# KMS-TEAM/vi_slam

Measured on AMD Instinct MI355X. Metric: frames/sec ORB extract+match, higher is better.
Workload: dtype u8; 1 GPU; kitti00_mono_1241x376_n1000; nfeatures=1000, nlevels=8, contexts_in_flight=4, distinct_frames=32, match=SearchForInitialization(prev frame) window 100

## Files before the change

vi_slam_amd/csrc/vslam_ctx.h:

```cpp
#ifndef VSLAM_CTX_H
#define VSLAM_CTX_H
#include <hip/hip_runtime.h>

#include <algorithm>
#include <atomic>
#include <cmath>
#include <condition_variable>
#include <cstdio>
#include <cstring>
#include <functional>
#include <mutex>
#include <string>
#include <thread>
#include <vector>

#include "../../include/vslam_orb_pattern.h"
#include "vslam_host.h"
#include "vslam_pool.h"
#include "vslam_kernels.h"
#include "vslam_tuning.h"

std::string& vslam_err();
#define g_err (vslam_err())

// ... 159 lines not shown
    double rgbd_ms = 0;
    long rgbd_passes = 0;
    hipEvent_t ev_lp[3] = {};
    bool lp_timed = false;
    double lp_ms[2] = {0, 0};
    long lp_passes = 0;

    bool dev_octree = false;
    OctParams oct;
    uint32_t* d_pts = nullptr;
    uint8_t* d_oct_sorted = nullptr;
    uint32_t* d_oct_lut = nullptr;
    int32_t* d_oct_redo = nullptr;
    uint32_t* d_sel_xyr = nullptr;
    int32_t* d_sel_cnt = nullptr;
    int32_t* d_counts = nullptr;
    int32_t* h_counts = nullptr;
    bool cand_on_host = false;
    int last_nimg = 0;

    bool profiling = false;
    hipEvent_t ev_prof[10] = {};
    double prof_ms[5] = {0, 0, 0, 0, 0};
    long prof_batches = 0, prof_images = 0;

    WorkerPool* pool = nullptr;
};


static inline int vslam_pix_bpp(int fmt) { return fmt == VSLAM_PIX_GRAY8 ? 1 : fmt <= VSLAM_PIX_BGR8 ? 3 : 4; }
// ... 44 lines not shown
```

vi_slam_amd/csrc/vslam_device.h:

```cpp
#ifndef VSLAM_DEVICE_H
#define VSLAM_DEVICE_H

#include <hip/hip_runtime.h>
#include <stdint.h>

#include "../../include/vslam_fe.h"

#define VSLAM_EDGE 19
#define VSLAM_BORDER 16
#define VSLAM_HALF_PATCH 15

struct LevelGeom {
    int32_t w, h;
    int32_t pitch;
    uint32_t off;
    float scale;
    int32_t pad[3];
};

struct PyramidGeom {
    int32_t nlevels;
    int32_t pad[3];
    LevelGeom lv[VSLAM_MAX_LEVELS];
};
// ... 33 lines not shown
    int32_t nIni[VSLAM_MAX_LEVELS];
    float hX[VSLAM_MAX_LEVELS];
    int32_t cellFirst[VSLAM_MAX_LEVELS + 1];
    int32_t selOff[VSLAM_MAX_LEVELS];
    int32_t selStride;
    int32_t maxNodes;
    int32_t ptsCap;
    int32_t maxIter;
    void* dbg;
    int32_t fineD[VSLAM_MAX_LEVELS];
    int32_t lutOff[VSLAM_MAX_LEVELS];
    int32_t lutW[VSLAM_MAX_LEVELS];
    int32_t fineLdsOff;
    int32_t fineLdsBytes;
    const uint32_t* lut;
};

struct StereoJob {
    const vslam_kp* kpsL;
    const uint8_t* descL;
    const vslam_kp* kpsR;
    const uint8_t* descR;
    const int32_t* cntL;
    const int32_t* cntR;
    int32_t slotL, slotR;
};
#define VSLAM_MAX_STEREO_JOBS 32
struct StereoJobs {
    StereoJob job[VSLAM_MAX_STEREO_JOBS];
};
// ... 169 lines not shown
```

vi_slam_amd/csrc/vslam_fe.hip:

```cpp
#if defined(__SSE2__)
#include <emmintrin.h>
#endif
#include "vslam_ctx.h"

#include <algorithm>
#include <chrono>
#include <mutex>
#include <cstdio>
#include <cstdlib>

void vslam_host_prof_report();

std::string& vslam_err() {
    static thread_local std::string e;
    return e;
}
extern "C" const char* vslam_last_error(void) { return vslam_err().c_str(); }

static std::mutex g_gate_mu;

static void gate_unlink(vslam_fe* fe) {
    if (fe->fast_gate) {
        auto& w = fe->fast_gate->gate_waiters;
        w.erase(std::remove(w.begin(), w.end(), fe), w.end());
// ... 29 lines not shown
    hipFree(fe->d_pattern);
    if (fe->h_top2) hipHostFree(fe->h_top2);
    hipFree(fe->d_part);
    hipFree(fe->d_idx2);
    hipFree(fe->d_dist2);
    hipFree(fe->d_dmat);
    hipFree(fe->d_tmp_desc[0]);
    hipFree(fe->d_tmp_desc[1]);
    hipFree(fe->d_stereo);
    hipFree(fe->d_pts);
    hipFree(fe->d_oct_sorted);
    hipFree(fe->d_oct_lut);
    hipFree(fe->d_sel_xyr);
    hipFree(fe->d_oct_redo);
    hipFree(fe->d_sel_cnt);
    if (fe->h_stereo) hipHostFree(fe->h_stereo);
    if (!fe->init_in_block) hipFree(fe->d_init);
    hipFree(fe->d_init_scratch);
    hipFree(fe->d_ukps);
    hipFree(fe->d_proj);
    hipFree(fe->d_sbp);
    if (fe->h_sbp) hipHostFree(fe->h_sbp);
    hipFree(fe->d_x3dw);
    hipFree(fe->d_mpflags);
    if (fe->h_proj) hipHostFree(fe->h_proj);
    if (fe->h_img) hipHostFree(fe->h_img);
    if (fe->h_depth) hipHostFree(fe->h_depth);
    hipFree(fe->d_stage);
    if (fe->graph_exec) hipGraphExecDestroy(fe->graph_exec);
    hipFree(fe->d_bow);
// ... 274 lines not shown
    fe->oct_threads = fe->tune.oct_threads == 256 || fe->tune.oct_threads == 512 || fe->tune.oct_threads == 1024
                          ? fe->tune.oct_threads
                          : fe->B <= 2 ? 1024 : 256;
    if (!on_device) return VSLAM_OK;
    if (vk_octree_set_max_lds((size_t)O.fineLdsOff + (size_t)O.fineLdsBytes + 16) != 0) {
        g_err = "hipFuncSetAttribute(k_octree, max dynamic LDS) failed";
        return VSLAM_ERR_HIP;
    }
    const size_t np = (size_t)fe->B * fe->cand_cap;
    HIPCHK(hipMalloc((void**)&fe->d_pts, np * 4));
    HIPCHK(hipMalloc((void**)&fe->d_sel_xyr, (size_t)fe->B * O.selStride * 4));
    HIPCHK(hipMalloc((void**)&fe->d_sel_cnt, (size_t)fe->B * VSLAM_MAX_LEVELS * 4));
    HIPCHK(hipMalloc((void**)&fe->d_oct_sorted, np * 8));
    HIPCHK(hipMalloc((void**)&fe->d_oct_redo, (size_t)fe->B * VSLAM_MAX_LEVELS * 4));
    HIPCHK(hipMemset(fe->d_oct_redo, 0, (size_t)fe->B * VSLAM_MAX_LEVELS * 4));
    UPLOAD(fe->d_oct_lut, plan.lut.data(), plan.lut.size() * 4);
    O.lut = fe->d_oct_lut;
    return VSLAM_OK;
}

static int create_stream_and_pool(vslam_fe* fe) {
    const int pr = tune_or(fe->tune.stream_priority, 0);
    int lo = 0, hi = 0;
    if (pr != 0 && hipDeviceGetStreamPriorityRange(&lo, &hi) == hipSuccess && lo != hi)
        HIPCHK(hipStreamCreateWithPriority(&fe->stream, hipStreamNonBlocking, pr == 1 ? lo : hi));
    else
        HIPCHK(hipStreamCreateWithFlags(&fe->stream, hipStreamNonBlocking));
    HIPCHK(hipEventCreateWithFlags(&fe->ev_cand, hipEventDisableTiming));
    fe->use_graph = fe->tune.graphs != 0;
    fe->sel_level.resize((size_t)fe->B * fe->p.nlevels);
// ... 397 lines not shown
        if (fe->pix_fmt != VSLAM_PIX_GRAY8) {
            vk_gray_images(st, ds, fe->d_pyr, fe->slot_stride, fe->geom.lv[0].off, fe->geom.lv[0].pitch, p.width, p.height, nimg,
                           0, fe->pix_fmt, fe->gray_shift, fe->tune);
            src_at_slots(fe, nimg);
        }
    } else {
        if (on_device != VSLAM_IMGS_STAGED) {
            int rc = upload_host_rows(fe, nimg, imgs, pitch, on_device);
            if (rc) return rc;
        }
        src_at_slots(fe, nimg);
    }
    fe->last_nimg = nimg;
    fe->cand_on_host = false;
    int32_t* d_errw = fe->dev_octree ? fe->d_counts + (size_t)fe->B * 4 : nullptr;
    if (fe->pyr_groups.empty()) vk_reset_headers(st, fe->d_cand, fe->cand_stride, nimg, d_errw);
    const bool prof = fe->profiling;
    if (prof) HIPCHK(hipEventRecord(fe->ev_prof[0], st));
    bool first_group = true;
    for (const auto& g : fe->pyr_groups) {
        vk_pyramid_group(st, fe->d_pyr, fe->slot_stride, fe->src, g.dev, g.lds_bytes, nimg,
                         first_group ? fe->d_cand : nullptr, fe->cand_stride, first_group ? d_errw : nullptr);
        first_group = false;
    }
    for (int l = 1; l < L && fe->pyr_groups.empty(); l++) {
        if (fe->d_quads[l])
            vk_resize_level_v2(st, fe->d_pyr, fe->slot_stride, fe->src, fe->geom.lv[l - 1], fe->geom.lv[l], l - 1,
                               fe->d_qbase[l], fe->d_quads[l], fe->d_ytab[l], fe->d_yb[l], nimg);
        else
            vk_resize_level(st, fe->d_pyr, fe->slot_stride, fe->src, fe->geom.lv[l - 1], fe->geom.lv[l], l - 1,
                            fe->d_xtab[l], fe->d_xa[l], fe->d_ytab[l], fe->d_yb[l], nimg);
    }
    if (prof) HIPCHK(hipEventRecord(fe->ev_prof[1], st));
    if (fe->fast_gate && fe->fast_gate->ev_fast) HIPCHK(hipStreamWaitEvent(st, fe->fast_gate->ev_fast, 0));
    if (fe->nbands > 0 && tune_or(fe->tune.fast_kernel, fe->B <= 2 ? 3 : 4) != 3)
        vk_fast_bands(st, fe->d_pyr, fe->slot_stride, fe->src, fe->geom, fe->d_bands, fe->nbands, fe->d_band_classes, fe->d_cells,
                      (int)fe->cells.size(), fe->d_cand, fe->cand_stride, p.ini_th_fast, p.min_th_fast, fe->band_max_wh, fe->band_max_iw, nimg);
// ... 91 lines not shown
    HIPCHK(hipMemcpyAsync(fe->d_counts, fe->h_counts, (size_t)(fe->B * 4 + 4) * 4, hipMemcpyHostToDevice, st));
    HIPCHK(hipMemcpyAsync(fe->d_sel, fe->h_sel, (size_t)nimg * fe->cap * sizeof(SelKp), hipMemcpyHostToDevice, st));
    if (fe->profiling) {
        HIPCHK(hipEventRecord(fe->ev_prof[7], st));
        HIPCHK(hipEventRecord(fe->ev_prof[8], st));
    }
    return VSLAM_OK;
}

static int select_dev(vslam_fe* fe, int nimg, int lap0, int lap1) {
    hipStream_t st = fe->stream;
    int32_t* d_err = fe->d_counts + (size_t)fe->B * 4;
    const int rc = enqueue_blur(fe, nimg);
    if (rc) return rc;
    if (fe->profiling) HIPCHK(hipEventRecord(fe->ev_prof[7], st));
    vk_octree(st, fe->d_cand, fe->cand_stride, (int)fe->cells.size(), fe->oct, fe->d_pts,
              fe->d_oct_sorted, (size_t)fe->cand_cap, fe->d_sel_xyr, fe->d_sel_cnt, d_err, fe->p.nlevels, nimg,
              fe->d_oct_redo, fe->tune.oct_regkeys, fe->oct_threads);
    vk_assign_out(st, fe->oct, fe->geom, fe->d_sel_xyr, fe->d_sel_cnt, lap0, lap1, fe->d_sel, fe->d_counts, fe->cap,
                  d_err, nimg, fe->d_oct_redo);
    if (fe->profiling) HIPCHK(hipEventRecord(fe->ev_prof[8], st));
    return VSLAM_OK;
}

static int enqueue_back(vslam_fe* fe, int nimg, int lap0, int lap1) {
    hipStream_t st = fe->stream;
    const bool prof = fe->profiling;
    int rc = fe->dev_octree ? select_dev(fe, nimg, lap0, lap1) : select_host(fe, nimg, lap0, lap1);
    if (rc) return rc;
    if (prof) HIPCHK(hipEventRecord(fe->ev_prof[5], st));
    vk_orient_describe_dev(st, fe->d_pyr, fe->d_blur, fe->slot_stride, fe->src, fe->geom, fe->d_sel, fe->d_counts,
                           fe->d_pattern, fe->d_kps, fe->d_desc, fe->cap, (fe->p.flags & VSLAM_FLAG_ATAN_FMA) ? 1 : 0,
                           nimg, fe->tune.desc_kpw >= 0 ? fe->tune.desc_kpw : fe->desc_kpw_hint);
    rc = vslam_enqueue_undistort(fe, nimg);
    if (rc) return rc;
// ... 610 lines not shown
```

vi_slam_amd/csrc/vslam_image_kernels.hip:

```cpp
#include "vslam_kernels.h"
#include "vslam_wave.h"

__device__ __forceinline__ const uint8_t* level_base_v2(const uint8_t* pyr, size_t slot_stride,
                                                        const BatchSrc& src, const LevelGeom& lg, int level,
                                                        int slot, int* pitch) {
    if (level == 0) {
        *pitch = (int)src.pitch0[slot];
        return src.l0[slot];
    }
    *pitch = lg.pitch;
    return pyr + (size_t)slot * slot_stride + lg.off;
}

__device__ __forceinline__ int refl101_v2(int p, int len) {
    if (p < 0) p = -p;
    if (p >= len) p = 2 * (len - 1) - p;
    return min(max(p, 0), len - 1);
}

#define BV_OUTW 248

__device__ __forceinline__ uint32_t udot4(uint32_t a, uint32_t b, uint32_t c) {
    return __builtin_amdgcn_udot4(a, b, c, false);
}
// ... 281 lines not shown
};
__device__ __forceinline__ PyrTileU pyr_tile_uniform(const PyrTileDev& t) {
    PyrTileU u;
#define PTU(f) u.f = __builtin_amdgcn_readfirstlane((int)t.f)
    PTU(c0); PTU(nc); PTU(r0); PTU(nr); PTU(sq0); PTU(sq1); PTU(sr0); PTU(sr1);
#undef PTU
    u.lds_off = (uint32_t)__builtin_amdgcn_readfirstlane((int)t.lds_off);
    u.pitch = (uint32_t)__builtin_amdgcn_readfirstlane((int)t.pitch);
    u.rt_off = (uint32_t)__builtin_amdgcn_readfirstlane((int)t.rt_off);
    return u;
}

template <int NT>
__global__ void __launch_bounds__(NT)
k_pyramid_group(uint8_t* pyr, size_t slot_stride, BatchSrc src, PyrGroupDev G, int nslots, uint8_t* reset_cand,
                size_t cand_stride, int32_t* reset_err) {
    extern __shared__ __align__(16) uint8_t psm[];
    constexpr int NW = NT / 64;
    const int lane = threadIdx.x & 63;
    const int wave = __builtin_amdgcn_readfirstlane((int)(threadIdx.x >> 6));
    if (reset_cand && blockIdx.x == 0) {
        if ((int)threadIdx.x < nslots) *(uint2*)(reset_cand + (size_t)threadIdx.x * cand_stride) = make_uint2(0u, 0u);
        if (reset_err && threadIdx.x < 4) reset_err[threadIdx.x] = 0;
    }
    const int nwork = G.ntiles * nslots, per_xcd = (nwork + 7) >> 3;
    const int wk = (int)(blockIdx.x & 7) * per_xcd + (int)(blockIdx.x >> 3);
    if (wk >= nwork) return;
    const int slot = wk / G.ntiles, tile = wk - slot * G.ntiles;
    const PyrTileDev* T = G.tiles + (size_t)tile * (G.nl + 1);
    const PyrTileDev S0 = T[0];
    if (S0.nr <= 0 || S0.nc <= 0) return;

    uint4 qsel[VSLAM_PYR_GROUP_LEVELS], qcf[VSLAM_PYR_GROUP_LEVELS];
    int qloc[VSLAM_PYR_GROUP_LEVELS];
#pragma unroll
    for (int j = 1; j <= VSLAM_PYR_GROUP_LEVELS; j++) {
        qsel[j - 1] = qcf[j - 1] = make_uint4(0, 0, 0, 0);
        qloc[j - 1] = 0;
// ... 89 lines not shown
                const uint32_t v0 = (uint32_t)(((__mul24(b0, g0) >> 16) + (__mul24(b1, hp0) >> 16) + 2) >> 2);
                const uint32_t v1 = (uint32_t)(((__mul24(b0, g1) >> 16) + (__mul24(b1, hp1) >> 16) + 2) >> 2);
                const uint32_t v2 = (uint32_t)(((__mul24(b0, g2) >> 16) + (__mul24(b1, hp2) >> 16) + 2) >> 2);
                const uint32_t v3 = (uint32_t)(((__mul24(b0, g3) >> 16) + (__mul24(b1, hp3) >> 16) + 2) >> 2);
                const uint32_t out = (v0 & 0xFF) | ((v1 & 0xFF) << 8) | ((v2 & 0xFF) << 16) | (v3 << 24);
                *(uint32_t*)(psm + dbase + __mul24(r, dp)) = out;
                if (qstore && r >= D.sr0 && r < D.sr1) *(uint32_t*)(gout + (size_t)r * gpitch) = out;
            }
#undef PYR_HPASS
        }
        __syncthreads();
    }
}

void vk_pyramid_group(hipStream_t st, uint8_t* pyr, size_t slot_stride, const BatchSrc& src, const PyrGroupDev& G,
                      size_t lds_bytes, int nslots, uint8_t* reset_cand, size_t cand_stride, int32_t* reset_err) {
    const int nwork = G.ntiles * nslots;
    hipLaunchKernelGGL(k_pyramid_group<256>, dim3(((nwork + 7) / 8) * 8), dim3(256), lds_bytes, st, pyr, slot_stride, src, G, nslots,
                       reset_cand, cand_stride, reset_err);
}

typedef unsigned short ushort2v __attribute__((ext_vector_type(2)));
__device__ __forceinline__ uint32_t pk_sub_sat(uint32_t a, uint32_t b) {
    uint32_t r;
    asm("v_pk_sub_u16 %0, %1, %2 clamp" : "=v"(r) : "v"(a), "v"(b));
    return r;
}
__device__ __forceinline__ uint32_t pk_add(uint32_t a, uint32_t b) {
    uint32_t r;
    asm("v_pk_add_u16 %0, %1, %2" : "=v"(r) : "v"(a), "v"(b));
    return r;
}
__device__ __forceinline__ uint32_t pk_min(uint32_t a, uint32_t b) {
    uint32_t r;
// ... 783 lines not shown
```

vi_slam_amd/csrc/vslam_kernels.h:

```cpp
#ifndef VSLAM_KERNELS_H
#define VSLAM_KERNELS_H

#include "vslam_tuning.h"
#include "vslam_device.h"

void vk_upload_disc(const int umax[16]);

void vk_resize_level(hipStream_t st, uint8_t* pyr, size_t slot_stride, const BatchSrc& src,
                     const LevelGeom& sg, const LevelGeom& dg, int src_level, const uint16_t* xtab,
                     const int16_t* xa, const uint16_t* ytab, const int16_t* yb, int nslots);

void vk_hamming_matrix(hipStream_t st, const uint8_t* q, int nq, const uint8_t* t, int nt, uint8_t* out);
int vk_hamming_top2_batch_split(int nprob, int max_nq, int max_nt);
void vk_hamming_top2_batch(hipStream_t st, const Top2Jobs& jobs, int nprob, int max_nq, int nrows, int nsplit, uint32_t* part,
                           int32_t* idx2, int32_t* dist2);

void vk_blur7_v2(hipStream_t st, const uint8_t* pyr, size_t slot_stride, const BatchSrc& src, const PyramidGeom& g,
                 uint8_t* blur, const uint32_t* tasks, int ntasks, const int32_t taps[7], int rows_per_task,
                 int nslots);
void vk_pyramid_group(hipStream_t st, uint8_t* pyr, size_t slot_stride, const BatchSrc& src, const PyrGroupDev& G,
                      size_t lds_bytes, int nslots, uint8_t* reset_cand = nullptr, size_t cand_stride = 0,
                      int32_t* reset_err = nullptr);
void vk_fast_cells_v3(hipStream_t st, const uint8_t* pyr, size_t slot_stride, const BatchSrc& src,
                      const PyramidGeom& g, const CellDesc* cells, int ncells, uint8_t* cand_region,
                      size_t cand_stride, int iniTh, int minTh, int tile_rows, int max_window_w, int max_px, int nslots);
int vk_fast_bands_check(int max_wh, int max_iw, int max_cells_per_band);
void vk_fast_bands(hipStream_t st, const uint8_t* pyr, size_t slot_stride, const BatchSrc& src, const PyramidGeom& g,
                   const BandDesc* bands, int nbands, const uint8_t* classes, const CellDesc* cells, int ncells, uint8_t* cand_region,
                   size_t cand_stride, int iniTh, int minTh, int max_wh, int max_iw, int nslots);
void vk_resize_level_v2(hipStream_t st, uint8_t* pyr, size_t slot_stride, const BatchSrc& src, const LevelGeom& sg,
                        const LevelGeom& dg, int src_level, const uint16_t* qbase, const ResizeQuad* quads,
                        const uint16_t* ytab, const int16_t* yb, int nslots);
size_t vk_octree_lds_bytes(int maxNodes);
int vk_octree_set_max_lds(size_t bytes);
void vk_octree(hipStream_t st, const uint8_t* cand_region, size_t cand_stride, int ncells, const OctParams& P,
               uint32_t* keys_a, void* sorted_a, size_t pts_stride,
               uint32_t* sel_xyr, int32_t* sel_cnt, int32_t* err_flag, int nlevels, int nslots, int32_t* deep_flags,
               int regkeys, int threads = 1024);
void vk_assign_out(hipStream_t st, const OctParams& P, const PyramidGeom& g, uint32_t* sel_xyr, int32_t* sel_cnt, int lap0,
                   int lap1, SelKp* sel, int32_t* slot_counts, int cap, int32_t* err_flag, int nslots,
                   const int32_t* deep_flags);
void vk_orient_describe_dev(hipStream_t st, const uint8_t* pyr, const uint8_t* blur, size_t slot_stride,
                            const BatchSrc& src, const PyramidGeom& g, const SelKp* sel,
                            const int32_t* slot_counts, const int8_t* pattern, vslam_kp* kps, uint8_t* desc,
                            int cap, int atan_fma, int nslots, int kpw_override = -1);

void vk_dbg_sincos(hipStream_t st, const float* x, int n, float* s, float* c);
void vk_dbg_logf(hipStream_t st, const float* x, int n, float* y);
void vk_dbg_atan2(hipStream_t st, const float* y, const float* x, int n, int fma, float* a);

void vk_stereo(hipStream_t st, const StereoJobs& jobs, int njobs, int maxNL, int maxNR, const PyramidGeom& g,
               const uint8_t* pyrL, size_t strideL, const BatchSrc& srcL, const uint8_t* pyrR, size_t strideR,
               const BatchSrc& srcR, float mbf, float maxD, uint32_t* best, float* uRight, float* depth,
               int32_t* sad, int cap, int max_band, uint8_t* rows_scratch);
size_t vk_stereo_rows_bytes(int njobs, int nrows, int max_band, int cap);
void vk_hamming_matrix_batch(hipStream_t st, const MatJobs& jobs, int njobs, int maxr, int maxc, const int32_t* idx,
// ... 3 lines not shown
int vk_search_init_set_max_lds(size_t bytes);
void vk_search_init(hipStream_t st, const InitJobs& jobs, int npairs, int cap, const SiBounds& bounds, int window,
                    float nnratio, int checkOri, int32_t* matches_out, float* prev_out, int32_t* nmatch_out,
                    int max_c2, int M, uint8_t* scratch, int* fallbacks, const vslam_tuning& T);
size_t vk_sbp_rank_lds(int nCur);
size_t vk_sbp_replay_lds(int nCur, int nLast);
size_t vk_sbp_scratch_bytes(int nLast, int M);
size_t vk_sbp_proj_bytes(int nLast);
int vk_sbp_set_max_lds(size_t bytes);
void vk_search_by_projection(hipStream_t st, const SbpJobs& JS, int njobs, int maxLast, int maxCur, int* fallbacks,
                             int forceSeq);
int vk_distinctive_set_max_lds(size_t bytes);
void vk_distinctive(hipStream_t st, const uint8_t* desc, const int32_t* offsets, int nsets, int maxN, int32_t* best);
void vk_unproject_stereo(hipStream_t st, const UnprojJobs& U, int njobs);
void vk_fuse_search(hipStream_t st, const FuseArgsDev& A);
void vk_reset_headers(hipStream_t st, uint8_t* d_cand, size_t cand_stride_bytes, int nimg, int32_t* d_err);
int vk_copy_ranges(hipStream_t st, const CopyRanges& R, const vslam_tuning& T = vslam_process_tuning());
void vk_undistort_kps(hipStream_t st, const vslam_kp* kps, const int32_t* counts, vslam_kp* ukps, int cap, int nimg,
                      const UdCam& cam);
void vk_undistort_xy(hipStream_t st, const float* xy, int n, float* out, const UdCam& cam);
void vk_pull_images(hipStream_t st, const BatchSrc& src, uint8_t* pyr, size_t slot_stride, uint32_t off0, int dpitch,
                    int w, int h, int nimg, int from_host, const vslam_tuning& T);
void vk_gray_images(hipStream_t st, const BatchSrc& src, uint8_t* pyr, size_t slot_stride, uint32_t off0, int dpitch, int w,
                    int h, int nimg, int from_host, int fmt, int shift, const vslam_tuning& T);
void vk_rgbd_depth(hipStream_t st, const vslam_kp* kps, const vslam_kp* ukps, const int32_t* counts, int cap, int nimg,
                   const RgbdDepthSrc& D, float* u_right, float* depth);
struct FrustumArgsDev;
struct FrustumCompactDev;
void vk_frustum(hipStream_t st, const FrustumArgsDev& A);
void vk_frustum_compact(hipStream_t st, const FrustumCompactDev& A);
void vk_pack_slots(hipStream_t st, const vslam_kp* kps, const uint8_t* desc, const int32_t* counts, int cap, int first,
// ... 5 lines not shown
```

vi_slam_amd/csrc/vslam_match_kernels.hip:

```cpp
#include "vslam_kernels.h"
#include "vslam_wave.h"
#include <cstring>
#include <cstdlib>

__device__ __forceinline__ const uint8_t* level_base2(const uint8_t* pyr, size_t slot_stride,
                                                      const BatchSrc& src, const LevelGeom& lg, int level,
                                                      int slot, int* pitch) {
    if (level == 0) {
        *pitch = (int)src.pitch0[slot];
        return src.l0[slot];
    }
    *pitch = lg.pitch;
    return pyr + (size_t)slot * slot_stride + lg.off;
}

#define JNL(j) (*(j).cntL)
#define JNR(j) (*(j).cntR)

__device__ __forceinline__ int refl101(int p, int len) {
    if (p < 0) p = -p;
    if (p >= len) p = 2 * (len - 1) - p;
    return min(max(p, 0), len - 1);
}

// ... 621 lines not shown
        const uint8_t* row = (const uint8_t*)D.img[s] + (size_t)v * D.pitch;
        d = D.type == VSLAM_DEPTH_F32 ? ((const float*)row)[u] : (float)((const uint16_t*)row)[u];
        if (D.scale) d = __fmul_rn(d, D.factor);
    }
    const bool ok = d > 0.0f;
    depth[at] = ok ? d : -1.0f;
    u_right[at] = ok ? __fsub_rn(ukps[at].x, __fdiv_rn(D.bf, d)) : -1.0f;
}

void vk_rgbd_depth(hipStream_t st, const vslam_kp* kps, const vslam_kp* ukps, const int32_t* counts, int cap, int nimg,
                   const RgbdDepthSrc& D, float* u_right, float* depth) {
    if (nimg <= 0 || cap <= 0) return;
    hipLaunchKernelGGL(k_rgbd_depth, dim3((cap + 255) / 256, nimg), dim3(256), 0, st, kps, ukps, counts, cap, D, u_right, depth);
}

__global__ void k_reset_headers(uint8_t* d_cand, size_t stride, int nimg, int32_t* d_err) {
    const int t = threadIdx.x;
    if (t < nimg) *(uint2*)(d_cand + (size_t)t * stride) = make_uint2(0u, 0u);
    if (d_err && t < 4) d_err[t] = 0;
}

void vk_reset_headers(hipStream_t st, uint8_t* d_cand, size_t cand_stride_bytes, int nimg, int32_t* d_err) {
    hipLaunchKernelGGL(k_reset_headers, dim3(1), dim3(64), 0, st, d_cand, cand_stride_bytes, nimg, d_err);
}

__global__ void __launch_bounds__(256)
k_distinctive(const uint8_t* __restrict__ desc, const int32_t* __restrict__ offsets, int32_t* __restrict__ best) {
    extern __shared__ __align__(16) uint8_t dsm[];
    uint4* sd = (uint4*)dsm;
    __shared__ uint32_t s_best;
    const int set = blockIdx.x, tid = threadIdx.x;
    const int o = offsets[set], N = offsets[set + 1] - o;
    if (N <= 0) {
        if (tid == 0) best[set] = -1;
        return;
    }
    for (int i = tid; i < 2 * N; i += 256) sd[i] = ((const uint4*)desc)[(size_t)o * 2 + i];
    if (tid == 0) s_best = 0xFFFFFFFFu;
// ... 32 lines not shown
```

vi_slam_amd/csrc/vslam_octree_kernel.hip:

```cpp
#include "vslam_kernels.h"

#include <mutex>

#ifndef O4BATCH
#define O4BATCH 8
#endif
typedef unsigned long long u64;

struct ONode {
    int16_t x0, y0, x1, y1;
    uint32_t begin;
    uint32_t cf;
};
#define ND_NOMORE(nd) ((nd).cf & 1u)

#define FB 21
#define FMASK ((1ull << FB) - 1)
__device__ __forceinline__ unsigned long long onehot(int q) { return q < 3 ? 1ull << (FB * q) : 0ull; }
__device__ __forceinline__ uint32_t fld(unsigned long long v, int q) { return (uint32_t)((v >> (FB * q)) & FMASK); }
__device__ __forceinline__ uint32_t nchildren(unsigned long long c, uint32_t count) {
    const uint32_t c0 = fld(c, 0), c1 = fld(c, 1), c2 = fld(c, 2);
    return (c0 != 0) + (c1 != 0) + (c2 != 0) + (count - c0 - c1 - c2 != 0);
}

// ... 50 lines not shown

__device__ __forceinline__ u64 deep_child_counts(const uint2* sorted, const uint32_t* PS, uint32_t path, int depth, int D,
                                                 float hX, int nIni, int Hh) {
    u64 c = 0ull;
    const uint32_t f = path >> (2 * (depth - D));
    for (uint32_t j = PS[f]; j < PS[f + 1]; j++) {
        const uint32_t kp = oct_key_path(sorted[j].x, hX, nIni, Hh, depth + 1);
        if ((kp >> 2) == path) c += onehot((int)(kp & 3u));
    }
    return c;
}

#define OCT_BEST(key, pos) ((((key) >> 24) << 20) | (0xFFFFFu - (uint32_t)(pos)))
#define OCT_BEST_POS(b) (0xFFFFFu - ((b) & 0xFFFFFu))

template <int OTV>
__global__ void __launch_bounds__(OTV)
k_octree_v4(const uint8_t* __restrict__ cand_region, size_t cand_stride, int ncells, OctParams P, uint32_t* keys_a,
            uint2* sorted_a, size_t pts_stride, uint32_t* sel_xyr, int32_t* sel_cnt, int32_t* err_flag,
            int32_t* deep_flags) {
    extern __shared__ __align__(16) uint8_t osm[];
    const int MAXN = P.maxNodes;
    ONode* cur = (ONode*)osm;
    ONode* nxt = cur + MAXN;
    uint32_t* Kq = (uint32_t*)(nxt + MAXN);
    u64* Cnt = (u64*)(nxt + MAXN) + MAXN;
    uint16_t* cb = (uint16_t*)(Cnt + MAXN);
    uint16_t* newIdx = cb + MAXN;
    uint16_t* prank = newIdx + MAXN;
    uint16_t* ordv = prank + MAXN;
    __shared__ uint32_t s_w32[OTV / 64];
    __shared__ int s_size, s_M, s_nexp, s_cut, s_deep;

    const int tid = threadIdx.x, lane = tid & 63, wv = tid >> 6;
    const int level = blockIdx.y, slot = blockIdx.x;
    const int N = P.N[level];
    const uint32_t* hdr = (const uint32_t*)(cand_region + (size_t)slot * cand_stride);
    const CellOut* cout = (const CellOut*)(hdr + 2);
    const uint32_t* cand = (const uint32_t*)(cout + ncells);
    uint32_t* pa = keys_a + (size_t)slot * pts_stride;
    uint2* sorted = sorted_a + (size_t)slot * pts_stride;
    uint32_t* out = sel_xyr + (size_t)slot * P.selStride + P.selOff[level];
    int32_t* ocnt = sel_cnt + slot * VSLAM_MAX_LEVELS + level;
    if (tid == 0) {
        deep_flags[slot * VSLAM_MAX_LEVELS + level] = 0;
        s_deep = 0;
    }
#ifdef VSLAM_OCT_STAMPS
    int dbgn3 = 0;
    unsigned long long* DBG3 = (unsigned long long*)P.dbg;
#ifndef VSLAM_OCT_STAMP_LEVEL
#define VSLAM_OCT_STAMP_LEVEL 0
#endif
#define STAMP3() do { if (DBG3 && tid == 0 && level == VSLAM_OCT_STAMP_LEVEL && slot == 0 && dbgn3 < 60) DBG3[dbgn3++] = __builtin_amdgcn_s_memrealtime(); } while (0)
#else
#define STAMP3() do { } while (0)
#endif
    STAMP3();

    const int c0 = P.cellFirst[level], c1 = P.cellFirst[level + 1];
    uint32_t off0 = 0;
    if (c0 > 0) {
// ... 1 lines not shown
        for (int c = tid; c < c0; c += OTV) before += cout[c].count;
        uint32_t tot;
        block_excl_scan<uint32_t, OTV>(before, s_w32, &tot);
        off0 = tot;
    }
    const int ncl = c1 - c0, K = (ncl + OTV - 1) / OTV;
    uint32_t mine = 0;
    for (int k = 0; k < K; k++) {
        const int c = c0 + tid * K + k;
        if (c < c1) mine += cout[c].count;
    }
    uint32_t ntot;
    uint32_t woff = block_excl_scan<uint32_t, OTV>(mine, s_w32, &ntot);
    const int n = (int)ntot;
    if (off0 + ntot > (uint32_t)P.ptsCap || n >= (1 << 20) || hdr[1] != 0) {
        if (tid == 0) {
            atomicOr(err_flag, 1);
            *ocnt = 0;
        }
        return;
    }
    pa += off0;
    sorted += off0;
    uint32_t* coff = (uint32_t*)nxt;
    uint32_t* cbas = coff + ncl + 1;
    for (int k = 0; k < K; k++) {
        const int c = c0 + tid * K + k;
        if (c < c1) {
            const CellOut co = cout[c];
            coff[c - c0] = woff;
            cbas[c - c0] = co.base;
            woff += co.count;
        }
    }
    if (tid == 0) coff[ncl] = ntot;
    if (n == 0) {
        if (tid == 0) *ocnt = 0;
        return;
    }
    const int nIni = P.nIni[level];
    const float hX = P.hX[level];
    const int Hh = P.H[level];
    const int D = P.fineD[level];
    const int cells = nIni << (2 * D);
    uint32_t* PS = (uint32_t*)(osm + P.fineLdsOff);
    uint32_t* Bst = PS + cells + 1;
    const uint32_t* __restrict__ xs = P.lut + P.lutOff[level];
    const uint32_t* __restrict__ ys = xs + P.lutW[level];
    for (int i = tid; i <= cells; i += OTV) PS[i] = Bst[i] = 0u;
    uint32_t warm = 0u;
    if (tid * 16 < P.lutW[level] + Hh + 1) warm = xs[tid * 16];
    __syncthreads();
// ... 279 lines not shown
        uint32_t* win = (uint32_t*)nxt;
        for (int v0 = 0; v0 < size; v0 += OTV / 4) {
            const int v = v0 + (tid >> 2), sub = tid & 3;
            uint32_t best = 0u;
            if (v < size) {
                const ONode nd = cur[v];
                const int sh = 2 * (D - ND4_DEPTH(nd));
                const uint32_t lo = nd.begin << sh, hi = (nd.begin + 1u) << sh;
                for (uint32_t j = lo + (uint32_t)sub; j < hi; j += 4) best = max(best, Bst[j]);
            }
            best = max(best, (uint32_t)__shfl_xor((int)best, 1, 64));
            best = max(best, (uint32_t)__shfl_xor((int)best, 2, 64));
            if (v < size && sub == 0) win[v] = OCT_BEST_POS(best);
        }
        __syncthreads();
        for (int v = tid; v < size; v += OTV) out[v] = pa[win[v]];
    } else {
        for (int v0 = 0; v0 < size; v0 += OTV / 4) {
            const int v = v0 + (tid >> 2), sub = tid & 3;
            u64 best = 0ull;
            uint32_t bkey = 0u;
            if (v < size) {
                const ONode nd = cur[v];
                const int depth = ND4_DEPTH(nd);
                const uint32_t path = nd.begin;
                if (depth <= D) {
                    const uint32_t lo = PS[path << (2 * (D - depth))], hi = PS[(path + 1u) << (2 * (D - depth))];
                    for (uint32_t j0 = lo + (uint32_t)sub; j0 < hi; j0 += 16) {
                        uint2 r[4];
#pragma unroll
                        for (int u = 0; u < 4; u++) r[u] = j0 + 4 * u < hi ? sorted[j0 + 4 * u] : make_uint2(0u, 0xFFFFFFFFu);
// ... 17 lines not shown
                                bkey = r.x;
                            }
                        }
                    }
                }
            }
#pragma unroll
            for (int o = 1; o < 4; o <<= 1) {
                const u64 ob = __shfl_xor(best, o, 64);
                const uint32_t ok = __shfl_xor(bkey, o, 64);
                if (ob > best) {
                    best = ob;
                    bkey = ok;
                }
            }
            if (v < size && sub == 0) out[v] = bkey;
        }
    }
#ifdef VSLAM_OCT_STAMPS
    __syncthreads();
    STAMP3();
    if (DBG3 && tid == 0 && level == VSLAM_OCT_STAMP_LEVEL && slot == 0) DBG3[63] = dbgn3;
#endif
    if (tid == 0) {
        *ocnt = size;
        if (s_deep) deep_flags[slot * VSLAM_MAX_LEVELS + level] = 1;
    }
}

#define AO_T 256
__global__ void __launch_bounds__(AO_T)
k_assign_out(OctParams P, PyramidGeom g, uint32_t* sel_xyr, int32_t* sel_cnt,
             int lap0, int lap1, SelKp* sel, int32_t* slot_counts , int cap,
             int32_t* err_flag, const int32_t* deep_flags) {
    __shared__ uint32_t s_w32[AO_T / 64];
    __shared__ int s_lvl_off[VSLAM_MAX_LEVELS + 1];
    const int tid = threadIdx.x, slot = blockIdx.x;
    const int L = g.nlevels;
    uint32_t redo_mask = 0;
    if (deep_flags && tid == 0)
        for (int lv = 0; lv < L; lv++) redo_mask |= deep_flags[slot * VSLAM_MAX_LEVELS + lv] ? 1u << lv : 0u;
    if (tid == 0) {
        int acc = 0;
        for (int l = 0; l < L; l++) {
            s_lvl_off[l] = acc;
            acc += sel_cnt[slot * VSLAM_MAX_LEVELS + l];
        }
        s_lvl_off[L] = acc;
    }
    __syncthreads();
    const int nk = s_lvl_off[L];
    if (nk > cap) {
        if (tid == 0) {
            atomicOr(err_flag, 2);
            slot_counts[slot * 4] = 0;
            slot_counts[slot * 4 + 1] = 0;
            slot_counts[slot * 4 + 2] = (int32_t)redo_mask;
        }
        return;
    }
    const int Cc = (nk + AO_T - 1) / AO_T;
    const int i0 = min(tid * Cc, nk), i1 = min(i0 + Cc, nk);
    const uint32_t* base = sel_xyr + (size_t)slot * P.selStride;
    uint32_t lapc = 0;
    int l = 0;
    for (int i = i0; i < i1; i++) {
        while (i >= s_lvl_off[l + 1]) l++;
        const uint32_t p = base[P.selOff[l] + (i - s_lvl_off[l])];
        float px = (float)((int)(p & 0xFFF) + VSLAM_BORDER);
        if (l) px = __fmul_rn(px, g.lv[l].scale);
        lapc += (px >= (float)lap0 && px <= (float)lap1) ? 1u : 0u;
    }
    uint32_t laptot;
    uint32_t lapbefore = block_excl_scan<uint32_t, AO_T>(lapc, s_w32, &laptot);
    l = 0;
    for (int i = i0; i < i1; i++) {
        while (i >= s_lvl_off[l + 1]) l++;
        const uint32_t p = base[P.selOff[l] + (i - s_lvl_off[l])];
        const int lx = (int)(p & 0xFFF) + VSLAM_BORDER, ly = (int)((p >> 12) & 0xFFF) + VSLAM_BORDER;
        float px = (float)lx;
        if (l) px = __fmul_rn(px, g.lv[l].scale);
        const bool inlap = px >= (float)lap0 && px <= (float)lap1;
        SelKp k;
        k.x = (uint16_t)lx;
        k.y = (uint16_t)ly;
        k.level = (uint8_t)l;
        k.slot = (uint8_t)slot;
        k.response = (uint8_t)(p >> 24);
        k.pad = 0;
        k.out = inlap ? (uint32_t)(nk - 1 - (int)lapbefore) : (uint32_t)(i - (int)lapbefore);
        if (inlap) lapbefore++;
        sel[(size_t)slot * cap + i] = k;
    }
    if (tid == 0) {
        slot_counts[slot * 4] = nk;
        slot_counts[slot * 4 + 1] = nk - (int)laptot;
        slot_counts[slot * 4 + 2] = (int32_t)redo_mask;
    }
}

size_t vk_octree_lds_bytes(int maxNodes) { return (size_t)maxNodes * (16 + 16 + 8 + 8 + 2 + 2 + 2 + 2) + 64; }

void vk_octree(hipStream_t st, const uint8_t* cand_region, size_t cand_stride, int ncells, const OctParams& P,
               uint32_t* keys_a, void* sorted_a, size_t pts_stride,
               uint32_t* sel_xyr, int32_t* sel_cnt, int32_t* err_flag, int nlevels, int nslots, int32_t* deep_flags,
               int regkeys , int threads ) {
    const dim3 grid(nslots, nlevels);
    const bool rk = regkeys < 0 ? nslots <= 2 : regkeys == 1;
    const size_t lds = (size_t)P.fineLdsOff + (size_t)P.fineLdsBytes;
    const int th = rk ? 1024 : (threads == 256 || threads == 512) ? threads : 1024;
#define OCT4_LAUNCH(TH)                                                                                          \
    hipLaunchKernelGGL((k_octree_v4<TH>), grid, dim3(TH), lds, st, cand_region, cand_stride, ncells, P, keys_a, \
                       (uint2*)sorted_a, pts_stride, sel_xyr, sel_cnt, err_flag, deep_flags)
    if (th == 256) OCT4_LAUNCH(256);
    else if (th == 512) OCT4_LAUNCH(512);
    else OCT4_LAUNCH(1024);
#undef OCT4_LAUNCH
}

void vk_assign_out(hipStream_t st, const OctParams& P, const PyramidGeom& g, uint32_t* sel_xyr, int32_t* sel_cnt, int lap0,
                   int lap1, SelKp* sel, int32_t* slot_counts, int cap, int32_t* err_flag, int nslots,
                   const int32_t* deep_flags) {
    hipLaunchKernelGGL(k_assign_out, dim3(nslots), dim3(AO_T), 0, st, P, g, sel_xyr, sel_cnt, lap0, lap1, sel,
                       slot_counts, cap, err_flag, deep_flags);
}

int vk_octree_set_max_lds(size_t bytes) {
    static std::mutex mu;
    static size_t have_dev[64] = {0};
    std::lock_guard<std::mutex> lk(mu);
    int dev = 0;
    if (hipGetDevice(&dev) != hipSuccess || dev < 0 || dev >= 64) return (int)hipErrorInvalidDevice;
    size_t& have = have_dev[dev];
    if (bytes <= have) return 0;
    const void* fns[3] = {(const void*)k_octree_v4<1024>, (const void*)k_octree_v4<512>, (const void*)k_octree_v4<256>};
    for (int i = 0; i < 3; i++) {
        const int rc = (int)hipFuncSetAttribute(fns[i], hipFuncAttributeMaxDynamicSharedMemorySize, (int)bytes);
        if (rc) return rc;
    }
// ... 4 lines not shown
```

Before: 203,100 frames/s.

## Fuse assign-out into octree kernel via last-block-arrives ticket

Removes the separate k_assign_out launch. Each octree block (one per slot and level) now publishes its count and deep flag with agent-scope atomics, then takes a per-slot arrival ticket. The last block to arrive computes the level offsets with a wave scan and writes the SelKp output. This trims one kernel launch and its dependency gap from the per-batch chain. In exchange it adds a per-slot arrival counter that must be reset (done in the pyramid and reset-header kernels), plus cross-block memory-ordering logic that has to be correct.

```diff
diff --git a/vi_slam_amd/csrc/vslam_ctx.h b/vi_slam_amd/csrc/vslam_ctx.h
--- a/vi_slam_amd/csrc/vslam_ctx.h
+++ b/vi_slam_amd/csrc/vslam_ctx.h
@@ -197,6 +197,7 @@
     int32_t* d_oct_redo = nullptr;
     uint32_t* d_sel_xyr = nullptr;
     int32_t* d_sel_cnt = nullptr;
+    int32_t* d_oct_arrive = nullptr;
     int32_t* d_counts = nullptr;
     int32_t* h_counts = nullptr;
     bool cand_on_host = false;
diff --git a/vi_slam_amd/csrc/vslam_device.h b/vi_slam_amd/csrc/vslam_device.h
--- a/vi_slam_amd/csrc/vslam_device.h
+++ b/vi_slam_amd/csrc/vslam_device.h
@@ -71,6 +71,16 @@
     int32_t fineLdsOff;
     int32_t fineLdsBytes;
     const uint32_t* lut;
+};
+
+struct OctTail {
+    int32_t lap0, lap1;
+    int32_t cap;
+    int32_t nlevels;
+    float scale[VSLAM_MAX_LEVELS];
+    SelKp* sel;
+    int32_t* slot_counts;
+    int32_t* arrive;
 };
 
 struct StereoJob {
diff --git a/vi_slam_amd/csrc/vslam_fe.hip b/vi_slam_amd/csrc/vslam_fe.hip
--- a/vi_slam_amd/csrc/vslam_fe.hip
+++ b/vi_slam_amd/csrc/vslam_fe.hip
@@ -67,6 +67,7 @@
     hipFree(fe->d_sel_xyr);
     hipFree(fe->d_oct_redo);
     hipFree(fe->d_sel_cnt);
+    hipFree(fe->d_oct_arrive);
     if (fe->h_stereo) hipHostFree(fe->h_stereo);
     if (!fe->init_in_block) hipFree(fe->d_init);
     hipFree(fe->d_init_scratch);
@@ -371,6 +372,8 @@
     HIPCHK(hipMalloc((void**)&fe->d_oct_sorted, np * 8));
     HIPCHK(hipMalloc((void**)&fe->d_oct_redo, (size_t)fe->B * VSLAM_MAX_LEVELS * 4));
     HIPCHK(hipMemset(fe->d_oct_redo, 0, (size_t)fe->B * VSLAM_MAX_LEVELS * 4));
+    HIPCHK(hipMalloc((void**)&fe->d_oct_arrive, (size_t)fe->B * 4));
+    HIPCHK(hipMemset(fe->d_oct_arrive, 0, (size_t)fe->B * 4));
     UPLOAD(fe->d_oct_lut, plan.lut.data(), plan.lut.size() * 4);
     O.lut = fe->d_oct_lut;
     return VSLAM_OK;
@@ -798,13 +801,15 @@
     fe->last_nimg = nimg;
     fe->cand_on_host = false;
     int32_t* d_errw = fe->dev_octree ? fe->d_counts + (size_t)fe->B * 4 : nullptr;
-    if (fe->pyr_groups.empty()) vk_reset_headers(st, fe->d_cand, fe->cand_stride, nimg, d_errw);
+    int32_t* d_arrive = fe->dev_octree ? fe->d_oct_arrive : nullptr;
+    if (fe->pyr_groups.empty()) vk_reset_headers(st, fe->d_cand, fe->cand_stride, nimg, d_errw, d_arrive);
     const bool prof = fe->profiling;
     if (prof) HIPCHK(hipEventRecord(fe->ev_prof[0], st));
     bool first_group = true;
     for (const auto& g : fe->pyr_groups) {
         vk_pyramid_group(st, fe->d_pyr, fe->slot_stride, fe->src, g.dev, g.lds_bytes, nimg,
-                         first_group ? fe->d_cand : nullptr, fe->cand_stride, first_group ? d_errw : nullptr);
+                         first_group ? fe->d_cand : nullptr, fe->cand_stride, first_group ? d_errw : nullptr,
+                         first_group ? d_arrive : nullptr);
         first_group = false;
     }
     for (int l = 1; l < L && fe->pyr_groups.empty(); l++) {
@@ -926,11 +931,18 @@
     const int rc = enqueue_blur(fe, nimg);
     if (rc) return rc;
     if (fe->profiling) HIPCHK(hipEventRecord(fe->ev_prof[7], st));
+    OctTail T;
+    T.lap0 = lap0;
+    T.lap1 = lap1;
+    T.cap = fe->cap;
+    T.nlevels = fe->p.nlevels;
+    for (int l = 0; l < VSLAM_MAX_LEVELS; l++) T.scale[l] = l < fe->geom.nlevels ? fe->geom.lv[l].scale : 1.0f;
+    T.sel = fe->d_sel;
+    T.slot_counts = fe->d_counts;
+    T.arrive = fe->d_oct_arrive;
     vk_octree(st, fe->d_cand, fe->cand_stride, (int)fe->cells.size(), fe->oct, fe->d_pts,
               fe->d_oct_sorted, (size_t)fe->cand_cap, fe->d_sel_xyr, fe->d_sel_cnt, d_err, fe->p.nlevels, nimg,
-              fe->d_oct_redo, fe->tune.oct_regkeys, fe->oct_threads);
-    vk_assign_out(st, fe->oct, fe->geom, fe->d_sel_xyr, fe->d_sel_cnt, lap0, lap1, fe->d_sel, fe->d_counts, fe->cap,
-                  d_err, nimg, fe->d_oct_redo);
+              fe->d_oct_redo, T, fe->tune.oct_regkeys, fe->oct_threads);
     if (fe->profiling) HIPCHK(hipEventRecord(fe->ev_prof[8], st));
     return VSLAM_OK;
 }
diff --git a/vi_slam_amd/csrc/vslam_image_kernels.hip b/vi_slam_amd/csrc/vslam_image_kernels.hip
--- a/vi_slam_amd/csrc/vslam_image_kernels.hip
+++ b/vi_slam_amd/csrc/vslam_image_kernels.hip
@@ -319,7 +319,7 @@
 template <int NT>
 __global__ void __launch_bounds__(NT)
 k_pyramid_group(uint8_t* pyr, size_t slot_stride, BatchSrc src, PyrGroupDev G, int nslots, uint8_t* reset_cand,
-                size_t cand_stride, int32_t* reset_err) {
+                size_t cand_stride, int32_t* reset_err, int32_t* reset_arrive) {
     extern __shared__ __align__(16) uint8_t psm[];
     constexpr int NW = NT / 64;
     const int lane = threadIdx.x & 63;
@@ -327,6 +327,7 @@
     if (reset_cand && blockIdx.x == 0) {
         if ((int)threadIdx.x < nslots) *(uint2*)(reset_cand + (size_t)threadIdx.x * cand_stride) = make_uint2(0u, 0u);
         if (reset_err && threadIdx.x < 4) reset_err[threadIdx.x] = 0;
+        if (reset_arrive && (int)threadIdx.x < nslots) reset_arrive[threadIdx.x] = 0;
     }
     const int nwork = G.ntiles * nslots, per_xcd = (nwork + 7) >> 3;
     const int wk = (int)(blockIdx.x & 7) * per_xcd + (int)(blockIdx.x >> 3);
@@ -446,10 +447,11 @@
 }
 
 void vk_pyramid_group(hipStream_t st, uint8_t* pyr, size_t slot_stride, const BatchSrc& src, const PyrGroupDev& G,
-                      size_t lds_bytes, int nslots, uint8_t* reset_cand, size_t cand_stride, int32_t* reset_err) {
+                      size_t lds_bytes, int nslots, uint8_t* reset_cand, size_t cand_stride, int32_t* reset_err,
+                      int32_t* reset_arrive) {
     const int nwork = G.ntiles * nslots;
     hipLaunchKernelGGL(k_pyramid_group<256>, dim3(((nwork + 7) / 8) * 8), dim3(256), lds_bytes, st, pyr, slot_stride, src, G, nslots,
-                       reset_cand, cand_stride, reset_err);
+                       reset_cand, cand_stride, reset_err, reset_arrive);
 }
 
 typedef unsigned short ushort2v __attribute__((ext_vector_type(2)));
diff --git a/vi_slam_amd/csrc/vslam_kernels.h b/vi_slam_amd/csrc/vslam_kernels.h
--- a/vi_slam_amd/csrc/vslam_kernels.h
+++ b/vi_slam_amd/csrc/vslam_kernels.h
@@ -20,7 +20,7 @@
                  int nslots);
 void vk_pyramid_group(hipStream_t st, uint8_t* pyr, size_t slot_stride, const BatchSrc& src, const PyrGroupDev& G,
                       size_t lds_bytes, int nslots, uint8_t* reset_cand = nullptr, size_t cand_stride = 0,
-                      int32_t* reset_err = nullptr);
+                      int32_t* reset_err = nullptr, int32_t* reset_arrive = nullptr);
 void vk_fast_cells_v3(hipStream_t st, const uint8_t* pyr, size_t slot_stride, const BatchSrc& src,
                       const PyramidGeom& g, const CellDesc* cells, int ncells, uint8_t* cand_region,
                       size_t cand_stride, int iniTh, int minTh, int tile_rows, int max_window_w, int max_px, int nslots);
@@ -36,10 +36,7 @@
 void vk_octree(hipStream_t st, const uint8_t* cand_region, size_t cand_stride, int ncells, const OctParams& P,
                uint32_t* keys_a, void* sorted_a, size_t pts_stride,
                uint32_t* sel_xyr, int32_t* sel_cnt, int32_t* err_flag, int nlevels, int nslots, int32_t* deep_flags,
-               int regkeys, int threads = 1024);
-void vk_assign_out(hipStream_t st, const OctParams& P, const PyramidGeom& g, uint32_t* sel_xyr, int32_t* sel_cnt, int lap0,
-                   int lap1, SelKp* sel, int32_t* slot_counts, int cap, int32_t* err_flag, int nslots,
-                   const int32_t* deep_flags);
+               const OctTail& T, int regkeys, int threads = 1024);
 void vk_orient_describe_dev(hipStream_t st, const uint8_t* pyr, const uint8_t* blur, size_t slot_stride,
                             const BatchSrc& src, const PyramidGeom& g, const SelKp* sel,
                             const int32_t* slot_counts, const int8_t* pattern, vslam_kp* kps, uint8_t* desc,
@@ -73,7 +70,8 @@
 void vk_distinctive(hipStream_t st, const uint8_t* desc, const int32_t* offsets, int nsets, int maxN, int32_t* best);
 void vk_unproject_stereo(hipStream_t st, const UnprojJobs& U, int njobs);
 void vk_fuse_search(hipStream_t st, const FuseArgsDev& A);
-void vk_reset_headers(hipStream_t st, uint8_t* d_cand, size_t cand_stride_bytes, int nimg, int32_t* d_err);
+void vk_reset_headers(hipStream_t st, uint8_t* d_cand, size_t cand_stride_bytes, int nimg, int32_t* d_err,
+                      int32_t* d_arrive = nullptr);
 int vk_copy_ranges(hipStream_t st, const CopyRanges& R, const vslam_tuning& T = vslam_process_tuning());
 void vk_undistort_kps(hipStream_t st, const vslam_kp* kps, const int32_t* counts, vslam_kp* ukps, int cap, int nimg,
                       const UdCam& cam);
diff --git a/vi_slam_amd/csrc/vslam_match_kernels.hip b/vi_slam_amd/csrc/vslam_match_kernels.hip
--- a/vi_slam_amd/csrc/vslam_match_kernels.hip
+++ b/vi_slam_amd/csrc/vslam_match_kernels.hip
@@ -659,14 +659,16 @@
     hipLaunchKernelGGL(k_rgbd_depth, dim3((cap + 255) / 256, nimg), dim3(256), 0, st, kps, ukps, counts, cap, D, u_right, depth);
 }
 
-__global__ void k_reset_headers(uint8_t* d_cand, size_t stride, int nimg, int32_t* d_err) {
+__global__ void k_reset_headers(uint8_t* d_cand, size_t stride, int nimg, int32_t* d_err, int32_t* d_arrive) {
     const int t = threadIdx.x;
     if (t < nimg) *(uint2*)(d_cand + (size_t)t * stride) = make_uint2(0u, 0u);
     if (d_err && t < 4) d_err[t] = 0;
-}
-
-void vk_reset_headers(hipStream_t st, uint8_t* d_cand, size_t cand_stride_bytes, int nimg, int32_t* d_err) {
-    hipLaunchKernelGGL(k_reset_headers, dim3(1), dim3(64), 0, st, d_cand, cand_stride_bytes, nimg, d_err);
+    if (d_arrive && t < nimg) d_arrive[t] = 0;
+}
+
+void vk_reset_headers(hipStream_t st, uint8_t* d_cand, size_t cand_stride_bytes, int nimg, int32_t* d_err,
+                      int32_t* d_arrive) {
+    hipLaunchKernelGGL(k_reset_headers, dim3(1), dim3(64), 0, st, d_cand, cand_stride_bytes, nimg, d_err, d_arrive);
 }
 
 __global__ void __launch_bounds__(256)
diff --git a/vi_slam_amd/csrc/vslam_octree_kernel.hip b/vi_slam_amd/csrc/vslam_octree_kernel.hip
--- a/vi_slam_amd/csrc/vslam_octree_kernel.hip
+++ b/vi_slam_amd/csrc/vslam_octree_kernel.hip
@@ -88,11 +88,113 @@
 #define OCT_BEST(key, pos) ((((key) >> 24) << 20) | (0xFFFFFu - (uint32_t)(pos)))
 #define OCT_BEST_POS(b) (0xFFFFFu - ((b) & 0xFFFFFu))
 
+#define OCT_PUB_ST(p, v) __hip_atomic_store((p), (v), __ATOMIC_RELAXED, __HIP_MEMORY_SCOPE_AGENT)
+#define OCT_PUB_LD(p) __hip_atomic_load((p), __ATOMIC_RELAXED, __HIP_MEMORY_SCOPE_AGENT)
+#define OCT_DRAIN_STORES() asm volatile("s_waitcnt vmcnt(0)" ::: "memory")
+
+template <int NT>
+__device__ __forceinline__ void oct_assign_out(const OctParams& P, const OctTail& T, const uint32_t* sel_xyr, int slot,
+                                               const int* lvl_off, uint32_t deep_mask, uint32_t* s_w32, int32_t* err_flag) {
+    const int tid = threadIdx.x;
+    const int L = T.nlevels, cap = T.cap, lap0 = T.lap0, lap1 = T.lap1;
+    const int nk = lvl_off[L];
+    if (nk > cap) {
+        if (tid == 0) {
+            atomicOr(err_flag, 2);
+            T.slot_counts[slot * 4] = 0;
+            T.slot_counts[slot * 4 + 1] = 0;
+            T.slot_counts[slot * 4 + 2] = (int32_t)deep_mask;
+        }
+        return;
+    }
+    const int Cc = (nk + NT - 1) / NT;
+    const int i0 = min(tid * Cc, nk), i1 = min(i0 + Cc, nk);
+    const uint32_t* base = sel_xyr + (size_t)slot * P.selStride;
+    uint32_t lapc = 0;
+    int l = 0;
+    for (int i = i0; i < i1; i++) {
+        while (i >= lvl_off[l + 1]) l++;
+        const uint32_t p = base[P.selOff[l] + (i - lvl_off[l])];
+        float px = (float)((int)(p & 0xFFF) + VSLAM_BORDER);
+        if (l) px = __fmul_rn(px, T.scale[l]);
+        lapc += (px >= (float)lap0 && px <= (float)lap1) ? 1u : 0u;
+    }
+    uint32_t laptot;
+    uint32_t lapbefore = block_excl_scan<uint32_t, NT>(lapc, s_w32, &laptot);
+    l = 0;
+    for (int i = i0; i < i1; i++) {
+        while (i >= lvl_off[l + 1]) l++;
+        const uint32_t p = base[P.selOff[l] + (i - lvl_off[l])];
+        const int lx = (int)(p & 0xFFF) + VSLAM_BORDER, ly = (int)((p >> 12) & 0xFFF) + VSLAM_BORDER;
+        float px = (float)lx;
+        if (l) px = __fmul_rn(px, T.scale[l]);
+        const bool inlap = px >= (float)lap0 && px <= (float)lap1;
+        SelKp k;
+        k.x = (uint16_t)lx;
+        k.y = (uint16_t)ly;
+        k.level = (uint8_t)l;
+        k.slot = (uint8_t)slot;
+        k.response = (uint8_t)(p >> 24);
+        k.pad = 0;
+        k.out = inlap ? (uint32_t)(nk - 1 - (int)lapbefore) : (uint32_t)(i - (int)lapbefore);
+        if (inlap) lapbefore++;
+        T.sel[(size_t)slot * cap + i] = k;
+    }
+    if (tid == 0) {
+        T.slot_counts[slot * 4] = nk;
+        T.slot_counts[slot * 4 + 1] = nk - (int)laptot;
+        T.slot_counts[slot * 4 + 2] = (int32_t)deep_mask;
+    }
+}
+
+template <int NT>
+__device__ __forceinline__ void oct_finish(const OctParams& P, const OctTail& T, const uint32_t* sel_xyr, int32_t* sel_cnt,
+                                           int32_t* deep_flags, int32_t* err_flag, int slot, int level, int size, int deep,
+                                           uint8_t* lds, uint32_t* s_w32) {
+    const int tid = threadIdx.x, L = T.nlevels;
+    int* lvl_off = (int*)lds;
+    int* tail = lvl_off + VSLAM_MAX_LEVELS + 1;
+    if (tid == 0) {
+        OCT_PUB_ST(sel_cnt + slot * VSLAM_MAX_LEVELS + level, size);
+        OCT_PUB_ST(deep_flags + slot * VSLAM_MAX_LEVELS + level, deep);
+    }
+    OCT_DRAIN_STORES();
+    __syncthreads();
+    if (tid == 0) {
+        const int ticket = __hip_atomic_fetch_add(T.arrive + slot, 1, __ATOMIC_RELAXED, __HIP_MEMORY_SCOPE_AGENT);
+        const int last = ticket == (int)gridDim.y - 1;
+        if (last) {
+            __builtin_amdgcn_fence(__ATOMIC_ACQUIRE, "agent");
+            OCT_DRAIN_STORES();
+            OCT_PUB_ST(T.arrive + slot, 0);
+        }
+        tail[0] = last;
+    }
+    __syncthreads();
+    if (!tail[0]) return;
+    if (tid < VSLAM_MAX_LEVELS) {
+        const int cnt = tid < L ? OCT_PUB_LD(sel_cnt + slot * VSLAM_MAX_LEVELS + tid) : 0;
+        const int dp = tid < L ? OCT_PUB_LD(deep_flags + slot * VSLAM_MAX_LEVELS + tid) : 0;
+        int inc = cnt;
+#pragma unroll
+        for (int o = 1; o < VSLAM_MAX_LEVELS; o <<= 1) {
+            const int t = __shfl_up(inc, o, 64);
+            if (tid >= o) inc += t;
+        }
+        lvl_off[tid] = inc - cnt;
+        if (tid == VSLAM_MAX_LEVELS - 1) lvl_off[VSLAM_MAX_LEVELS] = inc;
+        const unsigned long long m = __ballot(dp != 0);
+        if (tid == 0) tail[1] = (int)(uint32_t)m;
+    }
+    __syncthreads();
+    oct_assign_out<NT>(P, T, sel_xyr, slot, lvl_off, (uint32_t)tail[1], s_w32, err_flag);
+}
+
 template <int OTV>
 __global__ void __launch_bounds__(OTV)
 k_octree_v4(const uint8_t* __restrict__ cand_region, size_t cand_stride, int ncells, OctParams P, uint32_t* keys_a,
             uint2* sorted_a, size_t pts_stride, uint32_t* sel_xyr, int32_t* sel_cnt, int32_t* err_flag,
-            int32_t* deep_flags) {
+            int32_t* deep_flags, OctTail T) {
     extern __shared__ __align__(16) uint8_t osm[];
     const int MAXN = P.maxNodes;
     ONode* cur = (ONode*)osm;
@@ -115,11 +217,7 @@
     uint32_t* pa = keys_a + (size_t)slot * pts_stride;
     uint2* sorted = sorted_a + (size_t)slot * pts_stride;
     uint32_t* out = sel_xyr + (size_t)slot * P.selStride + P.selOff[level];
-    int32_t* ocnt = sel_cnt + slot * VSLAM_MAX_LEVELS + level;
-    if (tid == 0) {
-        deep_flags[slot * VSLAM_MAX_LEVELS + level] = 0;
-        s_deep = 0;
-    }
+    if (tid == 0) s_deep = 0;
 #ifdef VSLAM_OCT_STAMPS
     int dbgn3 = 0;
     unsigned long long* DBG3 = (unsigned long long*)P.dbg;
@@ -151,10 +249,8 @@
     uint32_t woff = block_excl_scan<uint32_t, OTV>(mine, s_w32, &ntot);
     const int n = (int)ntot;
     if (off0 + ntot > (uint32_t)P.ptsCap || n >= (1 << 20) || hdr[1] != 0) {
-        if (tid == 0) {
-            atomicOr(err_flag, 1);
-            *ocnt = 0;
-        }
+        if (tid == 0) atomicOr(err_flag, 1);
+        oct_finish<OTV>(P, T, sel_xyr, sel_cnt, deep_flags, err_flag, slot, level, 0, 0, osm, s_w32);
         return;
     }
     pa += off0;
@@ -172,7 +268,7 @@
     }
     if (tid == 0) coff[ncl] = ntot;
     if (n == 0) {
-        if (tid == 0) *ocnt = 0;
+        oct_finish<OTV>(P, T, sel_xyr, sel_cnt, deep_flags, err_flag, slot, level, 0, 0, osm, s_w32);
         return;
     }
     const int nIni = P.nIni[level];
@@ -482,7 +578,7 @@
             if (v < size && sub == 0) win[v] = OCT_BEST_POS(best);
         }
         __syncthreads();
-        for (int v = tid; v < size; v += OTV) out[v] = pa[win[v]];
+        for (int v = tid; v < size; v += OTV) OCT_PUB_ST(out + v, pa[win[v]]);
     } else {
         for (int v0 = 0; v0 < size; v0 += OTV / 4) {
             const int v = v0 + (tid >> 2), sub = tid & 3;
@@ -530,7 +626,7 @@
                     bkey = ok;
                 }
             }
-            if (v < size && sub == 0) out[v] = bkey;
+            if (v < size && sub == 0) OCT_PUB_ST(out + v, bkey);
         }
     }
 #ifdef VSLAM_OCT_STAMPS
@@ -538,81 +634,7 @@
     STAMP3();
     if (DBG3 && tid == 0 && level == VSLAM_OCT_STAMP_LEVEL && slot == 0) DBG3[63] = dbgn3;
 #endif
-    if (tid == 0) {
-        *ocnt = size;
-        if (s_deep) deep_flags[slot * VSLAM_MAX_LEVELS + level] = 1;
-    }
-}
-
-#define AO_T 256
-__global__ void __launch_bounds__(AO_T)
-k_assign_out(OctParams P, PyramidGeom g, uint32_t* sel_xyr, int32_t* sel_cnt,
-             int lap0, int lap1, SelKp* sel, int32_t* slot_counts , int cap,
-             int32_t* err_flag, const int32_t* deep_flags) {
-    __shared__ uint32_t s_w32[AO_T / 64];
-    __shared__ int s_lvl_off[VSLAM_MAX_LEVELS + 1];
-    const int tid = threadIdx.x, slot = blockIdx.x;
-    const int L = g.nlevels;
-    uint32_t redo_mask = 0;
-    if (deep_flags && tid == 0)
-        for (int lv = 0; lv < L; lv++) redo_mask |= deep_flags[slot * VSLAM_MAX_LEVELS + lv] ? 1u << lv : 0u;
-    if (tid == 0) {
-        int acc = 0;
-        for (int l = 0; l < L; l++) {
-            s_lvl_off[l] = acc;
-            acc += sel_cnt[slot * VSLAM_MAX_LEVELS + l];
-        }
-        s_lvl_off[L] = acc;
-    }
-    __syncthreads();
-    const int nk = s_lvl_off[L];
-    if (nk > cap) {
-        if (tid == 0) {
-            atomicOr(err_flag, 2);
-            slot_counts[slot * 4] = 0;
-            slot_counts[slot * 4 + 1] = 0;
-            slot_counts[slot * 4 + 2] = (int32_t)redo_mask;
-        }
-        return;
-    }
-    const int Cc = (nk + AO_T - 1) / AO_T;
-    const int i0 = min(tid * Cc, nk), i1 = min(i0 + Cc, nk);
-    const uint32_t* base = sel_xyr + (size_t)slot * P.selStride;
-    uint32_t lapc = 0;
-    int l = 0;
-    for (int i = i0; i < i1; i++) {
-        while (i >= s_lvl_off[l + 1]) l++;
-        const uint32_t p = base[P.selOff[l] + (i - s_lvl_off[l])];
-        float px = (float)((int)(p & 0xFFF) + VSLAM_BORDER);
-        if (l) px = __fmul_rn(px, g.lv[l].scale);
-        lapc += (px >= (float)lap0 && px <= (float)lap1) ? 1u : 0u;
-    }
-    uint32_t laptot;
-    uint32_t lapbefore = block_excl_scan<uint32_t, AO_T>(lapc, s_w32, &laptot);
-    l = 0;
-    for (int i = i0; i < i1; i++) {
-        while (i >= s_lvl_off[l + 1]) l++;
-        const uint32_t p = base[P.selOff[l] + (i - s_lvl_off[l])];
-        const int lx = (int)(p & 0xFFF) + VSLAM_BORDER, ly = (int)((p >> 12) & 0xFFF) + VSLAM_BORDER;
-        float px = (float)lx;
-        if (l) px = __fmul_rn(px, g.lv[l].scale);
-        const bool inlap = px >= (float)lap0 && px <= (float)lap1;
-        SelKp k;
-        k.x = (uint16_t)lx;
-        k.y = (uint16_t)ly;
-        k.level = (uint8_t)l;
-        k.slot = (uint8_t)slot;
-        k.response = (uint8_t)(p >> 24);
-        k.pad = 0;
-        k.out = inlap ? (uint32_t)(nk - 1 - (int)lapbefore) : (uint32_t)(i - (int)lapbefore);
-        if (inlap) lapbefore++;
-        sel[(size_t)slot * cap + i] = k;
-    }
-    if (tid == 0) {
-        slot_counts[slot * 4] = nk;
-        slot_counts[slot * 4 + 1] = nk - (int)laptot;
-        slot_counts[slot * 4 + 2] = (int32_t)redo_mask;
-    }
+    oct_finish<OTV>(P, T, sel_xyr, sel_cnt, deep_flags, err_flag, slot, level, size, s_deep, osm, s_w32);
 }
 
 size_t vk_octree_lds_bytes(int maxNodes) { return (size_t)maxNodes * (16 + 16 + 8 + 8 + 2 + 2 + 2 + 2) + 64; }
@@ -620,25 +642,19 @@
 void vk_octree(hipStream_t st, const uint8_t* cand_region, size_t cand_stride, int ncells, const OctParams& P,
                uint32_t* keys_a, void* sorted_a, size_t pts_stride,
                uint32_t* sel_xyr, int32_t* sel_cnt, int32_t* err_flag, int nlevels, int nslots, int32_t* deep_flags,
-               int regkeys , int threads ) {
+               const OctTail& T, int regkeys ,
+               int threads ) {
     const dim3 grid(nslots, nlevels);
     const bool rk = regkeys < 0 ? nslots <= 2 : regkeys == 1;
     const size_t lds = (size_t)P.fineLdsOff + (size_t)P.fineLdsBytes;
     const int th = rk ? 1024 : (threads == 256 || threads == 512) ? threads : 1024;
 #define OCT4_LAUNCH(TH)                                                                                          \
     hipLaunchKernelGGL((k_octree_v4<TH>), grid, dim3(TH), lds, st, cand_region, cand_stride, ncells, P, keys_a, \
-                       (uint2*)sorted_a, pts_stride, sel_xyr, sel_cnt, err_flag, deep_flags)
+                       (uint2*)sorted_a, pts_stride, sel_xyr, sel_cnt, err_flag, deep_flags, T)
     if (th == 256) OCT4_LAUNCH(256);
     else if (th == 512) OCT4_LAUNCH(512);
     else OCT4_LAUNCH(1024);
 #undef OCT4_LAUNCH
-}
-
-void vk_assign_out(hipStream_t st, const OctParams& P, const PyramidGeom& g, uint32_t* sel_xyr, int32_t* sel_cnt, int lap0,
-                   int lap1, SelKp* sel, int32_t* slot_counts, int cap, int32_t* err_flag, int nslots,
-                   const int32_t* deep_flags) {
-    hipLaunchKernelGGL(k_assign_out, dim3(nslots), dim3(AO_T), 0, st, P, g, sel_xyr, sel_cnt, lap0, lap1, sel,
-                       slot_counts, cap, err_flag, deep_flags);
 }
 
 int vk_octree_set_max_lds(size_t bytes) {
```

Result: no change. 202,400 frames/s, median of 2 (-0.3%).
